# lucidrains/audiolm-pytorch

Hardware: NVIDIA H100
Metric: CoarseTransformer tokens/sec fwd+bwd seq2048 (higher is better)
Workload: dtype bf16

## Files before the change

### audiolm_pytorch_b200/_lib.py

```python
from __future__ import annotations

import ctypes as C
import os
from pathlib import Path

import torch

_PKG = Path(__file__).resolve().parent
LIB_PATH = _PKG / "libalm_b200.so"

P = C.c_void_p
I = C.c_int
L = C.c_int64
F = C.c_float
U32 = C.c_uint32
U64 = C.c_uint64
DROP = [F, U64, U32]

SIGNATURES: dict[str, list] = {
    "alm_gemm_bf16": [P, I, L, L, P, I, L, L, P, I, L, L, I, I, I, I, F, P, I, I, P],
    "alm_mqa_attn_fwd": [P, L, P, L, L, P, L, L, P, P, L, P, L, P, L, L, I, I, I, I, I, F, *DROP, P],
    "alm_mqa_attn_bwd": [P, L, P, L, L, P, L, L, P, L, P, P, P, I, P, L, P, P, L, P, L, P, P, L, L, I, I, I, I, I, F, *DROP,
                         P],
    "alm_pack_key_mask": [P, P, I, I, P],
# ... 51 lines not shown
    "alm_sq_decode": [P, I, I, I, I, I, I, P, P, P, P, I, I, P, L, P],
    "alm_hubert_conv0": [P, P, P, P, I, I, I, I, I, P],
    "alm_hubert_chan_stats": [P, P, I, I, I, P],
    "alm_hubert_norm_act": [P, P, I, P, L, P, P, I, P, P, L, I, P],
    "alm_hubert_add_ln": [P, P, I, I, P, I, P, P, I, P, P, L, I, P],
    "alm_hubert_pos_pack": [P, P, I, I, I, I, I, I, P],
    "alm_hubert_qkv_heads": [P, P, P, P, I, I, I, I, P],
    "alm_hubert_merge_heads": [P, P, I, I, I, I, P],
}


class AlmError(RuntimeError):
    pass


_lib = None


def load() -> C.CDLL:
    global _lib
    if _lib is not None:
        return _lib
    if not LIB_PATH.exists():
        raise AlmError(
            f"{LIB_PATH} not found. Build it with `python -m audiolm_pytorch_b200.build` "
            "(there is no CPU / PyTorch fallback for the hot path)."
        )
    lib = C.CDLL(str(LIB_PATH), mode=os.RTLD_LOCAL | os.RTLD_NOW)
    lib.alm_version.restype = I
    lib.alm_status_string.restype = C.c_char_p
    lib.alm_status_string.argtypes = [I]
    lib.alm_launch_count.restype = C.c_ulonglong
    lib.alm_reset_launch_count.restype = None
    lib.alm_decode_stack_scratch_bytes.restype = L
    lib.alm_decode_stack_scratch_bytes.argtypes = [I, I, I, I]
    lib.alm_gemm_head_ce_tiles.restype = I
    lib.alm_gemm_head_ce_tiles.argtypes = [I]
    lib.alm_codec_gate_loop_workspace.restype = C.c_longlong
    lib.alm_codec_gate_loop_workspace.argtypes = [I, I, I, I]
    lib.alm_decode_stack_grid.restype = I
    lib.alm_decode_stack_grid.argtypes = []
    lib.alm_decode_stack_plan.restype = I
    lib.alm_decode_stack_plan.argtypes = [I, I, I, I, I, P]
    lib.alm_decode_stack_plan_dh.restype = I
    lib.alm_decode_stack_plan_dh.argtypes = [I, I, I, I, I, I, P]
    lib.alm_decode_stack_trace_offset.restype = L
    lib.alm_decode_stack_trace_offset.argtypes = [I, I, I, I]
    for name, argtypes in SIGNATURES.items():
        fn = getattr(lib, name)
        fn.argtypes = argtypes
        fn.restype = I
    _lib = lib
    return lib


def ptr(t) -> int | None:
    if t is None:
        return None
    return t.data_ptr()


def stream_handle() -> int:
    return torch.cuda.current_stream().cuda_stream


def call(name: str, *args) -> None:
    lib = load()
    conv = []
    for a in args:
        if isinstance(a, torch.Tensor):
            if not a.is_cuda:
                raise AlmError(f"{name}: got a {a.device} tensor; the hot path has no CPU implementation")
            conv.append(a.data_ptr())
        else:
            conv.append(a)
    rc = getattr(lib, name)(*conv, stream_handle())
    if rc != 0:
        raise AlmError(f"{name} failed: {lib.alm_status_string(rc).decode()} ({rc})")


def launch_count() -> int:
    return int(load().alm_launch_count())


def reset_launch_count() -> None:
    load().alm_reset_launch_count()
```

### audiolm_pytorch_b200/csrc/ffn_loss_misc.cu

```cuda
#include <stdlib.h>

#include "alm_common.cuh"

namespace alm {

constexpr int FF_THREADS = 256;
constexpr int FF_MAX_CHUNKS = 4;

__device__ __forceinline__ void unpack8b(const uint4& u, float (&f)[8]) {
  f[0] = bf16_lo(u.x); f[1] = bf16_hi(u.x); f[2] = bf16_lo(u.y); f[3] = bf16_hi(u.y);
  f[4] = bf16_lo(u.z); f[5] = bf16_hi(u.z); f[6] = bf16_lo(u.w); f[7] = bf16_hi(u.w);
}
__device__ __forceinline__ uint32_t pk2b(float a, float b) {
  __nv_bfloat162 v = __floats2bfloat162_rn(a, b);
  return *reinterpret_cast<uint32_t*>(&v);
}
__device__ __forceinline__ uint4 pack8b(const float (&f)[8]) {
  return make_uint4(pk2b(f[0], f[1]), pk2b(f[2], f[3]), pk2b(f[4], f[5]), pk2b(f[6], f[7]));
}

template <int N>
__device__ __forceinline__ void block_sum256(float (&v)[N], float* buf ) {
  const int lane = threadIdx.x & 31, warp = threadIdx.x >> 5;
#pragma unroll
  for (int i = 0; i < N; ++i) v[i] = warp_sum(v[i]);
  __syncthreads();
  if (lane == 0) {
#pragma unroll
    for (int i = 0; i < N; ++i) buf[i * 8 + warp] = v[i];
  }
  __syncthreads();
#pragma unroll
  for (int i = 0; i < N; ++i) {
    float s = 0.f;
#pragma unroll
// ... 17 lines not shown
#pragma unroll
  for (int i = 0; i < N; ++i) {
    float s = 0.f;
#pragma unroll
    for (int w = 0; w < NW; ++w) s += buf[i * NW + w];
    v[i] = s;
  }
}

__device__ __forceinline__ uint32_t row_keep_bits8(const DropoutArgs& d, uint32_t m, uint32_t c0) {
  const uint32_t hi = (c0 >> 3) & 1u;
  const uint32_t jb = c0 & ~15u;
  uint32_t own[4], other[4];
#pragma unroll
  for (int t = 0; t < 4; ++t) {
    own[t] = dropout_word(dropout_draw(d, m, jb + 4 * hi + t), m);
    other[t] = __shfl_xor_sync(0xffffffffu, own[t], 1);
  }
  uint32_t bits = 0;
#pragma unroll
  for (int e = 0; e < 8; ++e) {
    const uint32_t w = ((uint32_t)e >> 2) == hi ? own[e & 3] : other[e & 3];
    if (dropout_pick(d, make_uint4(w, w, w, w), m, c0 + e)) bits |= 1u << e;
  }
  return bits;
}

__device__ __forceinline__ float gelu_erf(float x) { return 0.5f * x * (1.f + erff(x * 0.7071067811865476f)); }

__device__ __forceinline__ float gelu_erf_grad(float x) {
  const float cdf = 0.5f * (1.f + erff(x * 0.7071067811865476f));
  const float pdf = 0.3989422804014327f * __expf(-0.5f * x * x);
  return cdf + x * pdf;
}

template <int NCH, int NT, bool DROPOUT>
__global__ void __launch_bounds__(NT)
geglu_ln_fwd_kernel(const __nv_bfloat16* __restrict__ h, long long ldh, int gate_off,
                    const float* __restrict__ gamma, __nv_bfloat16* __restrict__ gn, long long ldg,
                    float* __restrict__ stats, int M, int inner, int inner_pad, const DropoutArgs drop) {
  __shared__ float buf[2 * (NT / 32)];
  uint4 pa[NCH], pgt[NCH];
  auto load_row = [&](int row, uint4* xa, uint4* xg) {
#pragma unroll
    for (int k = 0; k < NCH; ++k) {
      const int c0 = (threadIdx.x + k * NT) * 8;
      if (c0 < inner_pad) {
        xa[k] = *reinterpret_cast<const uint4*>(h + (size_t)row * ldh + c0);
        xg[k] = *reinterpret_cast<const uint4*>(h + (size_t)row * ldh + gate_off + c0);
      }
    }
  };
  if ((int)blockIdx.x < M) load_row(blockIdx.x, pa, pgt);
  for (int m = blockIdx.x; m < M; m += gridDim.x) {
    uint4 na[NCH], ngt[NCH];
    if (m + (int)gridDim.x < M) load_row(m + gridDim.x, na, ngt);
    if (m + 2 * (int)gridDim.x < M && (threadIdx.x & 7) == 0) {
#pragma unroll
      for (int k = 0; k < NCH; ++k) {
        const int c0 = (threadIdx.x + k * NT) * 8;
        if (c0 < inner_pad) {
          asm volatile("prefetch.global.L2 [%0];" ::"l"(h + (size_t)(m + 2 * gridDim.x) * ldh + c0));
          asm volatile("prefetch.global.L2 [%0];" ::"l"(h + (size_t)(m + 2 * gridDim.x) * ldh + gate_off + c0));
        }
      }
    }
    float g[NCH][8];
    float s12[2] = {0.f, 0.f};
#pragma unroll
    for (int k = 0; k < NCH; ++k) {
      const int c0 = (threadIdx.x + k * NT) * 8;
#pragma unroll
      for (int e = 0; e < 8; ++e) g[k][e] = 0.f;
      if (c0 < inner_pad) {
        float a[8], gt[8];
        unpack8b(pa[k], a);
        unpack8b(pgt[k], gt);
        const int nv = min(8, inner - c0);
#pragma unroll
        for (int e = 0; e < 8; ++e) {
          float cdf, xpdf;
          gelu_parts(gt[e], cdf, xpdf);
          const float v = e < nv ? gt[e] * cdf * a[e] : 0.f;
          g[k][e] = v;
          s12[0] += v;
          s12[1] = fmaf(v, v, s12[1]);
        }
      }
    }
    block_sum_nt<2, NT>(s12, buf);
    const float mean = s12[0] / inner;
    const float rstd = rsqrtf(fmaxf(s12[1] / inner - mean * mean, 0.f) + 1e-5f);
#pragma unroll
    for (int k = 0; k < NCH; ++k) {
      const int c0 = (threadIdx.x + k * NT) * 8;
      [[maybe_unused]] uint32_t keep = 0;
      if constexpr (DROPOUT) keep = row_keep_bits8(drop, m, c0);
      if (c0 < inner_pad) {
        const int nv = min(8, inner - c0);
        float gm[8] = {0.f, 0.f, 0.f, 0.f, 0.f, 0.f, 0.f, 0.f};
        if (nv == 8) {
          const float4 g0 = __ldg(reinterpret_cast<const float4*>(gamma + c0));
          const float4 g1 = __ldg(reinterpret_cast<const float4*>(gamma + c0 + 4));
          gm[0] = g0.x; gm[1] = g0.y; gm[2] = g0.z; gm[3] = g0.w; gm[4] = g1.x; gm[5] = g1.y; gm[6] = g1.z; gm[7] = g1.w;
        } else {
#pragma unroll
          for (int e = 0; e < 8; ++e)
            if (e < nv) gm[e] = __ldg(gamma + c0 + e);
        }
        float o[8];
#pragma unroll
        for (int e = 0; e < 8; ++e) o[e] = e < nv ? (g[k][e] - mean) * rstd * gm[e] : 0.f;
        if constexpr (DROPOUT) {
#pragma unroll
          for (int e = 0; e < 8; ++e) o[e] = ((keep >> e) & 1u) ? o[e] * drop.scale : 0.f;
        }
        *reinterpret_cast<uint4*>(gn + (size_t)m * ldg + c0) = pack8b(o);
      }
    }
    if (threadIdx.x == 0) {
      stats[(size_t)m * 2] = mean;
      stats[(size_t)m * 2 + 1] = rstd;
    }
#pragma unroll
    for (int k = 0; k < NCH; ++k) { pa[k] = na[k]; pgt[k] = ngt[k]; }
  }
}

template <int NCH, int NT, bool DROPOUT>
__global__ void __launch_bounds__(NT, NT == 512 ? 2 : 1)
geglu_ln_bwd_kernel(const __nv_bfloat16* __restrict__ h, long long ldh, int gate_off,
                    const float* __restrict__ gamma, const float* __restrict__ stats,
                    const __nv_bfloat16* __restrict__ dgn, long long ldg, __nv_bfloat16* __restrict__ dh,
                    float* __restrict__ g_gamma, int M, int inner, int inner_pad, const DropoutArgs drop) {
  __shared__ float buf[2 * (NT / 32)];
  float gacc[NCH][8];
#pragma unroll
  for (int k = 0; k < NCH; ++k)
#pragma unroll
    for (int e = 0; e < 8; ++e) gacc[k][e] = 0.f;
  for (int m = blockIdx.x; m < M; m += gridDim.x) {
    if (m + (int)gridDim.x < M && (threadIdx.x & 7) == 0) {
#pragma unroll
      for (int k = 0; k < NCH; ++k) {
        const int c0 = (threadIdx.x + k * NT) * 8;
        if (c0 < inner_pad) {
          asm volatile("prefetch.global.L2 [%0];" ::"l"(h + (size_t)(m + gridDim.x) * ldh + c0));
          asm volatile("prefetch.global.L2 [%0];" ::"l"(h + (size_t)(m + gridDim.x) * ldh + gate_off + c0));
          asm volatile("prefetch.global.L2 [%0];" ::"l"(dgn + (size_t)(m + gridDim.x) * ldg + c0));
        }
      }
    }
    const float mean = stats[(size_t)m * 2], rstd = stats[(size_t)m * 2 + 1];
    float a[NCH][8], gp[NCH][8], gl[NCH][8], ge[NCH][8];
    float r2[2] = {0.f, 0.f};
#pragma unroll
    for (int k = 0; k < NCH; ++k) {
      const int c0 = (threadIdx.x + k * NT) * 8;
#pragma unroll
      for (int e = 0; e < 8; ++e) { a[k][e] = gp[k][e] = gl[k][e] = ge[k][e] = 0.f; }
      [[maybe_unused]] uint32_t keep = 0;
      if constexpr (DROPOUT) keep = row_keep_bits8(drop, m, c0);
      if (c0 < inner_pad) {
        float dv[8], gt[8];
        unpack8b(*reinterpret_cast<const uint4*>(h + (size_t)m * ldh + c0), a[k]);
        unpack8b(*reinterpret_cast<const uint4*>(h + (size_t)m * ldh + gate_off + c0), gt);
        unpack8b(*reinterpret_cast<const uint4*>(dgn + (size_t)m * ldg + c0), dv);
        if constexpr (DROPOUT) {
#pragma unroll
          for (int e = 0; e < 8; ++e) dv[e] = ((keep >> e) & 1u) ? dv[e] * drop.scale : 0.f;
        }
        const int nv = min(8, inner - c0);
        float gm[8] = {0.f, 0.f, 0.f, 0.f, 0.f, 0.f, 0.f, 0.f};
        if (nv == 8) {
          const float4 g0 = __ldg(reinterpret_cast<const float4*>(gamma + c0));
          const float4 g1 = __ldg(reinterpret_cast<const float4*>(gamma + c0 + 4));
          gm[0] = g0.x; gm[1] = g0.y; gm[2] = g0.z; gm[3] = g0.w; gm[4] = g1.x; gm[5] = g1.y; gm[6] = g1.z; gm[7] = g1.w;
        } else {
#pragma unroll
          for (int e = 0; e < 8; ++e)
            if (e < nv) gm[e] = __ldg(gamma + c0 + e);
        }
#pragma unroll
        for (int e = 0; e < 8; ++e) {
          float cdf, xpdf;
          gelu_parts(gt[e], cdf, xpdf);
          const bool ok = e < nv;
          ge[k][e] = ok ? gt[e] * cdf : 0.f;
          gp[k][e] = ok ? cdf + xpdf : 0.f;
          if (!ok) { a[k][e] = 0.f; dv[e] = 0.f; }
          const float xh = (ge[k][e] * a[k][e] - mean) * rstd;
          gl[k][e] = dv[e] * gm[e];
          gacc[k][e] = fmaf(dv[e], xh, gacc[k][e]);
          r2[0] += gl[k][e];
          r2[1] = fmaf(gl[k][e], xh, r2[1]);
        }
      }
    }
    block_sum_nt<2, NT>(r2, buf);
    const float m1 = r2[0] / inner, m2 = r2[1] / inner;
#pragma unroll
    for (int k = 0; k < NCH; ++k) {
      const int c0 = (threadIdx.x + k * NT) * 8;
      if (c0 < inner_pad) {
        const int nv = min(8, inner - c0);
        float da[8], dg8[8];
#pragma unroll
        for (int e = 0; e < 8; ++e) {
          const float xh = (ge[k][e] * a[k][e] - mean) * rstd;
          const float dg = e < nv ? rstd * (gl[k][e] - m1 - xh * m2) : 0.f;
          da[e] = dg * ge[k][e];
          dg8[e] = dg * a[k][e] * gp[k][e];
        }
        *reinterpret_cast<uint4*>(dh + (size_t)m * ldh + c0) = pack8b(da);
        *reinterpret_cast<uint4*>(dh + (size_t)m * ldh + gate_off + c0) = pack8b(dg8);
      }
    }
  }
#pragma unroll
  for (int k = 0; k < NCH; ++k) {
    const int c0 = (threadIdx.x + k * NT) * 8;
#pragma unroll
    for (int e = 0; e < 8; ++e)
      if (c0 + e < inner) atomicAdd(g_gamma + c0 + e, gacc[k][e]);
  }
}



__global__ void __launch_bounds__(FF_THREADS)
ce_fwd_bwd_kernel(const float* __restrict__ logits, long long ldl, const long long* __restrict__ labels,
                  long long ignore_index, float* __restrict__ loss_rows, __nv_bfloat16* __restrict__ dlogits,
                  long long ldd, const float* __restrict__ scale_num, const float* __restrict__ scale_den, int V,
                  int Vpad) {
  __shared__ float buf[2 * 8];
  const int r = blockIdx.x;
  const float* row = logits + (size_t)r * ldl;
  const long long label = labels[r];
  const bool ignored = (label == ignore_index);
  const bool bad_label = !ignored && (label < 0 || label >= V);
  float mx[1] = {-INFINITY};
  for (int c = threadIdx.x; c < V; c += FF_THREADS) mx[0] = fmaxf(mx[0], row[c]);
  {
    float v = warp_max(mx[0]);
    __syncthreads();
    if ((threadIdx.x & 31) == 0) buf[threadIdx.x >> 5] = v;
    __syncthreads();
    float m = buf[0];
#pragma unroll
    for (int w = 1; w < FF_THREADS / 32; ++w) m = fmaxf(m, buf[w]);
    mx[0] = m;
  }
  float sm[1] = {0.f};
  for (int c = threadIdx.x; c < V; c += FF_THREADS) sm[0] += __expf(row[c] - mx[0]);
  block_sum256<1>(sm, buf);
  const float lse = mx[0] + logf(sm[0]);
  const float nan = __int_as_float(0x7fc00000);
  if (threadIdx.x == 0) loss_rows[r] = ignored ? 0.f : bad_label ? nan : (lse - row[label]);
  if (dlogits != nullptr) {
    const float sc = ignored ? 0.f : bad_label ? nan : (*scale_num) / (*scale_den);
// ... 246 lines not shown
#pragma unroll
    for (int half = 0; half < 2; ++half) {
      const uint32_t c = j0 + 8 * half;
      if ((int)c >= C) continue;
      uint4* ptr = reinterpret_cast<uint4*>(x + (size_t)row * ld + c);
      float f[8];
      unpack8b(*ptr, f);
#pragma unroll
      for (int e = 0; e < 8; ++e) f[e] = dropout_pick(d, dr[e], row, c + e) ? f[e] * d.scale : 0.f;
      *ptr = pack8b(f);
    }
  }
}

}

using namespace alm;

extern "C" int alm_dropout_bf16(void* x, int64_t ld, int64_t M, int C, float p, uint64_t seed, uint32_t site,
                                alm_stream_t stream_) {
  cudaStream_t stream = reinterpret_cast<cudaStream_t>(stream_);
  ALM_REQUIRE(x && M >= 0 && C >= 0 && p >= 0.f && p < 1.f, ALM_ERR_ARG);
  ALM_REQUIRE(C % 8 == 0 && ld % 8 == 0 && ld >= C && (reinterpret_cast<uintptr_t>(x) & 15u) == 0, ALM_ERR_ALIGN);
  ALM_REQUIRE(M < (1ll << 32), ALM_ERR_UNSUPPORTED);
  if (M == 0 || C == 0 || p == 0.f) return ALM_OK;
  const long long threads = (M + 15) / 16 * 4 * ((C + 15) / 16);
  dropout_bf16_kernel<<<(unsigned)ceil_div(threads, 256LL), 256, 0, stream>>>(
      reinterpret_cast<__nv_bfloat16*>(x), ld, M, C, make_dropout_args(p, seed, site));
  ALM_CHECK_LAUNCH();
  ALM_LAUNCHED(1);
  return ALM_OK;
}

template <bool DROPOUT>
static void launch_geglu_ln_fwd(int nch, int grid, cudaStream_t stream, const __nv_bfloat16* hp, int64_t ldh,
                                int gate_off, const float* gamma, __nv_bfloat16* gp, int64_t ldg, float* stats, int M,
                                int inner, int inner_pad, const DropoutArgs& d) {
  if (nch <= 1) geglu_ln_fwd_kernel<1, 256, DROPOUT><<<grid, FF_THREADS, 0, stream>>>(hp, ldh, gate_off, gamma, gp, ldg, stats, M, inner, inner_pad, d);
  else if (nch == 2) geglu_ln_fwd_kernel<2, 256, DROPOUT><<<grid, FF_THREADS, 0, stream>>>(hp, ldh, gate_off, gamma, gp, ldg, stats, M, inner, inner_pad, d);
  else geglu_ln_fwd_kernel<4, 256, DROPOUT><<<grid, FF_THREADS, 0, stream>>>(hp, ldh, gate_off, gamma, gp, ldg, stats, M, inner, inner_pad, d);
}

extern "C" int alm_geglu_ln_fwd(const void* h, int64_t ldh, int gate_off, const float* gamma, void* gn, int64_t ldg,
                                float* stats, int M, int inner, int inner_pad, float dropout_p, uint64_t seed,
                                uint32_t site, alm_stream_t stream_) {
  cudaStream_t stream = reinterpret_cast<cudaStream_t>(stream_);
  ALM_REQUIRE(M > 0 && inner > 0 && inner_pad >= inner && inner_pad % 8 == 0, ALM_ERR_ARG);
  ALM_REQUIRE(dropout_p >= 0.f && dropout_p < 1.f, ALM_ERR_ARG);
  ALM_REQUIRE(ldh % 8 == 0 && ldg % 8 == 0 && gate_off % 8 == 0, ALM_ERR_ALIGN);
  const int nch = ceil_div(inner_pad / 8, FF_THREADS);
  ALM_REQUIRE(nch <= FF_MAX_CHUNKS, ALM_ERR_UNSUPPORTED);
  const int grid = min(M, num_sms() * 8);
  auto* hp = (const __nv_bfloat16*)h;
  auto* gp = (__nv_bfloat16*)gn;
  const DropoutArgs d = make_dropout_args(dropout_p, seed, site);
  if (dropout_p > 0.f) launch_geglu_ln_fwd<true>(nch, grid, stream, hp, ldh, gate_off, gamma, gp, ldg, stats, M, inner, inner_pad, d);
  else launch_geglu_ln_fwd<false>(nch, grid, stream, hp, ldh, gate_off, gamma, gp, ldg, stats, M, inner, inner_pad, d);
  ALM_CHECK_LAUNCH();
  ALM_LAUNCHED(1);
  return ALM_OK;
}

template <bool DROPOUT>
static void launch_geglu_ln_bwd(int nch, int threads, int grid, cudaStream_t stream, const __nv_bfloat16* hp,
                                int64_t ldh, int gate_off, const float* gamma, const float* stats,
                                const __nv_bfloat16* dg, int64_t ldg, __nv_bfloat16* dhp, float* g_gamma, int M,
                                int inner, int inner_pad, const DropoutArgs& d) {
  if (threads == 512) geglu_ln_bwd_kernel<1, 512, DROPOUT><<<grid, 512, 0, stream>>>(hp, ldh, gate_off, gamma, stats, dg, ldg, dhp, g_gamma, M, inner, inner_pad, d);
  else if (nch <= 1) geglu_ln_bwd_kernel<1, 256, DROPOUT><<<grid, FF_THREADS, 0, stream>>>(hp, ldh, gate_off, gamma, stats, dg, ldg, dhp, g_gamma, M, inner, inner_pad, d);
  else if (nch == 2) geglu_ln_bwd_kernel<2, 256, DROPOUT><<<grid, FF_THREADS, 0, stream>>>(hp, ldh, gate_off, gamma, stats, dg, ldg, dhp, g_gamma, M, inner, inner_pad, d);
  else geglu_ln_bwd_kernel<4, 256, DROPOUT><<<grid, FF_THREADS, 0, stream>>>(hp, ldh, gate_off, gamma, stats, dg, ldg, dhp, g_gamma, M, inner, inner_pad, d);
}

extern "C" int alm_geglu_ln_bwd(const void* h, int64_t ldh, int gate_off, const float* gamma, const float* stats,
                                const void* dgn, int64_t ldg, void* dh, float* g_gamma, int M, int inner,
                                int inner_pad, float dropout_p, uint64_t seed, uint32_t site, alm_stream_t stream_) {
  cudaStream_t stream = reinterpret_cast<cudaStream_t>(stream_);
  ALM_REQUIRE(M > 0 && inner > 0 && inner_pad >= inner && inner_pad % 8 == 0, ALM_ERR_ARG);
  ALM_REQUIRE(dropout_p >= 0.f && dropout_p < 1.f, ALM_ERR_ARG);
  ALM_REQUIRE(ldh % 8 == 0 && ldg % 8 == 0 && gate_off % 8 == 0, ALM_ERR_ALIGN);
  const int nch = ceil_div(inner_pad / 8, FF_THREADS);
  ALM_REQUIRE(nch <= FF_MAX_CHUNKS, ALM_ERR_UNSUPPORTED);
  auto* hp = (const __nv_bfloat16*)h;
  auto* dg = (const __nv_bfloat16*)dgn;
  auto* dhp = (__nv_bfloat16*)dh;
  static const int bwd_threads = getenv("ALM_GEGLU_BWD_THREADS") ? atoi(getenv("ALM_GEGLU_BWD_THREADS")) : 512;
  const int threads = bwd_threads == 512 && inner_pad > 2048 && inner_pad <= 4096 ? 512 : 256;
  const int grid = min(M, num_sms() * (threads == 512 ? 2 : 4));
  const DropoutArgs d = make_dropout_args(dropout_p, seed, site);
  if (dropout_p > 0.f) launch_geglu_ln_bwd<true>(nch, threads, grid, stream, hp, ldh, gate_off, gamma, stats, dg, ldg, dhp, g_gamma, M, inner, inner_pad, d);
  else launch_geglu_ln_bwd<false>(nch, threads, grid, stream, hp, ldh, gate_off, gamma, stats, dg, ldg, dhp, g_gamma, M, inner, inner_pad, d);
  ALM_CHECK_LAUNCH();
  ALM_LAUNCHED(1);
  return ALM_OK;
}

extern "C" int alm_ce_fwd_bwd(const float* logits, int64_t ldl, const int64_t* labels, int64_t ignore_index,
                              float* loss_rows, void* dlogits, int64_t ldd, const float* scale_num,
                              const float* scale_den, int rows, int V, int Vpad, alm_stream_t stream_) {
  cudaStream_t stream = reinterpret_cast<cudaStream_t>(stream_);
  ALM_REQUIRE(rows > 0 && V > 0 && Vpad >= V, ALM_ERR_ARG);
  ALM_REQUIRE(dlogits == nullptr || (scale_num && scale_den), ALM_ERR_ARG);
  ce_fwd_bwd_kernel<<<rows, FF_THREADS, 0, stream>>>(logits, ldl, (const long long*)labels, ignore_index,
                                                    loss_rows, (__nv_bfloat16*)dlogits, ldd, scale_num, scale_den, V,
                                                    Vpad);
  ALM_CHECK_LAUNCH();
  ALM_LAUNCHED(1);
  return ALM_OK;
}

extern "C" int alm_attn_delta_dh(const void* o, int64_t ldo, const void* d_o, int64_t lddo, float* delta,
                                 int64_t delta_stride, float* dq_acc, int b, int h, int n, int dim_head,
                                 alm_stream_t stream_) {
  cudaStream_t stream = reinterpret_cast<cudaStream_t>(stream_);
  ALM_REQUIRE(dim_head == 32 || dim_head == 64 || dim_head == 128, ALM_ERR_UNSUPPORTED);
  ALM_REQUIRE(b > 0 && h > 0 && n > 0, ALM_ERR_ARG);
  const long long warps = (long long)b * h * n;
  const int threads = 256;
  const long long blocks = ceil_div(warps * 32, (long long)threads);
  attn_delta_kernel<<<(unsigned)blocks, threads, 0, stream>>>((const __nv_bfloat16*)o, ldo,
                                                              (const __nv_bfloat16*)d_o, lddo, delta, delta_stride, dq_acc, b, h, n,
                                                              dim_head);
  ALM_CHECK_LAUNCH();
  ALM_LAUNCHED(1);
  return ALM_OK;
}

extern "C" int alm_attn_delta(const void* o, int64_t ldo, const void* d_o, int64_t lddo, float* delta,
// ... 128 lines not shown
```

### include/alm_b200.h

```cpp
#ifndef ALM_B200_H_
#define ALM_B200_H_

#include <stddef.h>
#include <stdint.h>

#ifdef __cplusplus
extern "C" {
#endif

typedef struct CUstream_st* alm_stream_t;

typedef enum alm_status {
  ALM_OK = 0,
  ALM_ERR_ARG = -1,
  ALM_ERR_ALIGN = -2,
  ALM_ERR_CUDA = -3,
  ALM_ERR_UNSUPPORTED = -4
} alm_status;

int alm_version(void);
const char* alm_status_string(int code);
unsigned long long alm_launch_count(void);
void alm_reset_launch_count(void);

// ... 78 lines not shown
                          float scale, int grid_ctas , alm_stream_t stream);

int alm_hc_pre_fwd(const void* R_in, const void* Y, const float* beta_prev, const float* x_expand,
                   const float* gamma_hc, const float* dyn_alpha, const float* dyn_beta, const float* static_alpha,
                   const float* static_beta, const float* alpha_scale, const float* beta_scale,
                   const float* ln_gamma, void* R_out, void* bin, void* xn, float* beta_out, float* aux, int M,
                   int d, int streams, alm_stream_t stream);
int alm_hc_pre_bwd(const void* R_in, const void* Y, const float* beta_prev, const float* x_expand,
                   const float* gamma_hc, const float* dyn_alpha, const float* dyn_beta, const float* static_alpha,
                   const float* static_beta, const float* alpha_scale, const float* beta_scale,
                   const float* ln_gamma, const float* aux, const void* dR_out, const void* dxn,
                   const void* dbin_extra, const float* dbeta, void* dR_in, void* dY, float* dbeta_prev,
                   float* dx_expand, float dx_scale, float* g_gamma_hc, float* g_dyn_alpha, float* g_dyn_beta,
                   float* g_static_alpha, float* g_static_beta, float* g_alpha_scale, float* g_beta_scale,
                   float* g_ln_gamma, int M, int d, int streams, alm_stream_t stream);
int alm_hc_post_fwd(const void* R_in, const void* Y, const float* beta_prev, const float* ln_gamma, void* out,
                    float* stats, int M, int d, int streams, alm_stream_t stream);
int alm_hc_post_bwd(const void* R_in, const void* Y, const float* beta_prev, const float* ln_gamma,
                    const float* stats, const void* dout, void* dR_in, void* dY, float* dbeta_prev,
                    float* g_ln_gamma, int M, int d, int streams, alm_stream_t stream);

int alm_resid_ln_fwd(const float* r, const void* y, const float* gamma, float* r_new, void* xn, void* rb, float* stats,
                     int M, int d, alm_stream_t stream);
int alm_resid_ln_bwd(const float* r_new, const float* gamma, const float* stats, const float* dr_out, const void* dxn,
                     const void* dextra, float* dr, void* dr_bf16, float* g_gamma, float out_scale, int M, int d,
                     alm_stream_t stream);

int alm_geglu_ln_fwd(const void* h, int64_t ldh, int gate_off, const float* gamma, void* gn, int64_t ldg,
                     float* stats, int M, int inner, int inner_pad, float dropout_p, uint64_t seed, uint32_t site,
                     alm_stream_t stream);
int alm_geglu_ln_bwd(const void* h, int64_t ldh, int gate_off, const float* gamma, const float* stats,
                     const void* dgn, int64_t ldg, void* dh, float* g_gamma, int M, int inner, int inner_pad,
                     float dropout_p, uint64_t seed, uint32_t site, alm_stream_t stream);

int alm_dropout_bf16(void* x, int64_t ld, int64_t M, int C, float p, uint64_t seed, uint32_t site,
                     alm_stream_t stream);

int alm_ce_fwd_bwd(const float* logits, int64_t ldl, const int64_t* labels, int64_t ignore_index, float* loss_rows,
                   void* dlogits, int64_t ldd, const float* scale_num, const float* scale_den, int rows, int V,
                   int Vpad, alm_stream_t stream);

int alm_topk_gumbel_sample(const float* logits, int64_t ldl, const float* uniform, int64_t ldu, int64_t* ids, int rows,
                           int V, int k, float temperature, alm_stream_t stream);

int alm_axpby_bf16(const void* x, int64_t ldx, float alpha, const void* y, int64_t ldy, float beta, void* out,
                   int64_t ldout, int64_t rows, int cols, alm_stream_t stream);
int alm_cast_pad_bf16(const float* src, int64_t lds, void* dst, int64_t ldd, int64_t rows, int cols, int cols_pad,
                      alm_stream_t stream);
int alm_cast_pad_multi(const int64_t* desc_dev, int n, alm_stream_t stream);
int alm_scale_by_scalar_bf16(void* x, const float* s, int64_t n, alm_stream_t stream);

int alm_causal_conv1d_fwd(const float* x, const float* w, const float* bias, const float* residual, float* y, int B,
                          int Cin, int Cout, int T, int K, int stride, int dilation, int pad_mode, int act_elu,
                          int w_packed, alm_stream_t stream);
int alm_residual_unit_fwd(const float* x, const float* w7_packed, const float* b7, const float* w1_packed,
                          const float* b1, float* y, int B, int C, int T, int dilation, int pad_mode,
                          alm_stream_t stream);
int alm_codec_se_fp32(const float* y, const float* x, const float* w1_folded, const float* b1, const float* w2,
                      const float* b2, float* out, int B, int C, int Ci, int T, alm_stream_t stream);
int alm_codec_first_conv(const float* x, const float* w, const float* bias, void* y, int B, int T, int Cout, int K,
                         int pad_mode, alm_stream_t stream);
int alm_codec_ru_tc(const void* x, void* y, const void* w_units, const float* b7, const float* b1, int B, int C, int T,
                    int dilation, int pad_mode, int out_phases, alm_stream_t stream);
int alm_codec_conv_tc(const void* x, void* y, const void* w_units, const float* bias, int B, int Cin, int Cout, int Tin,
                      int K, int stride, int pad_mode, int out_phases, int out_fp32, int upsample, alm_stream_t stream);
int alm_codec_ru_se_tc(const void* x, void* y, const void* w_units, const float* b7, const float* b1, const float* se_b1,
// ... 50 lines not shown
```

Before: 743,500.

## Add TMA bulk-copy ring-buffered persistent kernels for GEGLU+LayerNorm fwd/bwd

Adds persistent GEGLU+LayerNorm forward and backward kernels. Each prefetches whole input rows into a multi-stage shared-memory ring with cp.async.bulk and mbarriers, so the next rows' loads overlap compute on the current row. The old register-load kernels are refactored into shared device helpers and kept as a fallback, used for wide rows, small M, misaligned bases, or when an env var disables the ring. The ring adds shared-memory pressure and limits CTAs per SM, and a launch counter is exposed for inspection.

```diff
diff --git a/audiolm_pytorch_b200/_lib.py b/audiolm_pytorch_b200/_lib.py
--- a/audiolm_pytorch_b200/_lib.py
+++ b/audiolm_pytorch_b200/_lib.py
@@ -107,6 +107,7 @@
     lib.alm_status_string.argtypes = [I]
     lib.alm_launch_count.restype = C.c_ulonglong
     lib.alm_reset_launch_count.restype = None
+    lib.alm_geglu_ring_launches.restype = C.c_ulonglong
     lib.alm_decode_stack_scratch_bytes.restype = L
     lib.alm_decode_stack_scratch_bytes.argtypes = [I, I, I, I]
     lib.alm_gemm_head_ce_tiles.restype = I
@@ -160,3 +161,7 @@
 
 def reset_launch_count() -> None:
     load().alm_reset_launch_count()
+
+
+def geglu_ring_launches() -> int:
+    return int(load().alm_geglu_ring_launches())
diff --git a/audiolm_pytorch_b200/csrc/ffn_loss_misc.cu b/audiolm_pytorch_b200/csrc/ffn_loss_misc.cu
--- a/audiolm_pytorch_b200/csrc/ffn_loss_misc.cu
+++ b/audiolm_pytorch_b200/csrc/ffn_loss_misc.cu
@@ -1,6 +1,10 @@
 #include <stdlib.h>
+#include <string.h>
+
+#include <initializer_list>
 
 #include "alm_common.cuh"
+#include "ptx_sm90.cuh"
 
 namespace alm {
 
@@ -84,6 +88,103 @@
   const float cdf = 0.5f * (1.f + erff(x * 0.7071067811865476f));
   const float pdf = 0.3989422804014327f * __expf(-0.5f * x * x);
   return cdf + x * pdf;
+}
+
+
+__device__ __forceinline__ void load_gamma8(const float* __restrict__ gamma, int c0, int nv, float (&gm)[8]) {
+#pragma unroll
+  for (int e = 0; e < 8; ++e) gm[e] = 0.f;
+  if (nv == 8) {
+    const float4 g0 = __ldg(reinterpret_cast<const float4*>(gamma + c0));
+    const float4 g1 = __ldg(reinterpret_cast<const float4*>(gamma + c0 + 4));
+    gm[0] = g0.x; gm[1] = g0.y; gm[2] = g0.z; gm[3] = g0.w; gm[4] = g1.x; gm[5] = g1.y; gm[6] = g1.z; gm[7] = g1.w;
+  } else {
+#pragma unroll
+    for (int e = 0; e < 8; ++e)
+      if (e < nv) gm[e] = __ldg(gamma + c0 + e);
+  }
+}
+
+__device__ __forceinline__ void geglu_fwd_chunk(const uint4& ua, const uint4& ugt, int nv, float (&g)[8],
+                                                float (&s12)[2]) {
+  float a[8], gt[8];
+  unpack8b(ua, a);
+  unpack8b(ugt, gt);
+#pragma unroll
+  for (int e = 0; e < 8; ++e) {
+    float cdf, xpdf;
+    gelu_parts(gt[e], cdf, xpdf);
+    const float v = e < nv ? gt[e] * cdf * a[e] : 0.f;
+    g[e] = v;
+    s12[0] += v;
+    s12[1] = fmaf(v, v, s12[1]);
+  }
+}
+
+__device__ __forceinline__ void geglu_ln_stats(const float (&s12)[2], int inner, float& mean, float& rstd) {
+  mean = s12[0] / inner;
+  rstd = rsqrtf(fmaxf(fmaf(-mean, mean, s12[1] / inner), 0.f) + 1e-5f);
+}
+
+template <bool DROPOUT>
+__device__ __forceinline__ uint4 geglu_fwd_out(const float (&g)[8], const float* __restrict__ gamma, int c0, int nv,
+                                               float mean, float rstd, uint32_t keep, const DropoutArgs& drop) {
+  float gm[8];
+  load_gamma8(gamma, c0, nv, gm);
+  float o[8];
+#pragma unroll
+  for (int e = 0; e < 8; ++e) o[e] = e < nv ? (g[e] - mean) * rstd * gm[e] : 0.f;
+  if constexpr (DROPOUT) {
+#pragma unroll
+    for (int e = 0; e < 8; ++e) o[e] = ((keep >> e) & 1u) ? o[e] * drop.scale : 0.f;
+  }
+  return pack8b(o);
+}
+
+template <bool DROPOUT>
+__device__ __forceinline__ void geglu_bwd_chunk(const uint4& ua, const uint4& ugt, const uint4& udg, uint32_t keep,
+                                                const float* __restrict__ gamma, int c0, int nv, float mean,
+                                                float rstd, const DropoutArgs& drop, float (&a)[8], float (&ge)[8],
+                                                float (&gp)[8], float (&gl)[8], float (&gacc)[8], float (&r2)[2]) {
+  float dv[8], gt[8];
+  unpack8b(ua, a);
+  unpack8b(ugt, gt);
+  unpack8b(udg, dv);
+  if constexpr (DROPOUT) {
+#pragma unroll
+    for (int e = 0; e < 8; ++e) dv[e] = ((keep >> e) & 1u) ? dv[e] * drop.scale : 0.f;
+  }
+  float gm[8];
+  load_gamma8(gamma, c0, nv, gm);
+#pragma unroll
+  for (int e = 0; e < 8; ++e) {
+    float cdf, xpdf;
+    gelu_parts(gt[e], cdf, xpdf);
+    const bool ok = e < nv;
+    ge[e] = ok ? gt[e] * cdf : 0.f;
+    gp[e] = ok ? cdf + xpdf : 0.f;
+    if (!ok) { a[e] = 0.f; dv[e] = 0.f; }
+    const float xh = (ge[e] * a[e] - mean) * rstd;
+    gl[e] = dv[e] * gm[e];
+    gacc[e] = fmaf(dv[e], xh, gacc[e]);
+    r2[0] += gl[e];
+    r2[1] = fmaf(gl[e], xh, r2[1]);
+  }
+}
+
+__device__ __forceinline__ void geglu_bwd_out(const float (&a)[8], const float (&ge)[8], const float (&gp)[8],
+                                              const float (&gl)[8], int nv, float mean, float rstd, float m1, float m2,
+                                              uint4& da_out, uint4& dgt_out) {
+  float da[8], dg8[8];
+#pragma unroll
+  for (int e = 0; e < 8; ++e) {
+    const float xh = (ge[e] * a[e] - mean) * rstd;
+    const float dg = e < nv ? rstd * (gl[e] - m1 - xh * m2) : 0.f;
+    da[e] = dg * ge[e];
+    dg8[e] = dg * a[e] * gp[e];
+  }
+  da_out = pack8b(da);
+  dgt_out = pack8b(dg8);
 }
 
 template <int NCH, int NT, bool DROPOUT>
@@ -124,51 +225,19 @@
       const int c0 = (threadIdx.x + k * NT) * 8;
 #pragma unroll
       for (int e = 0; e < 8; ++e) g[k][e] = 0.f;
-      if (c0 < inner_pad) {
-        float a[8], gt[8];
-        unpack8b(pa[k], a);
-        unpack8b(pgt[k], gt);
-        const int nv = min(8, inner - c0);
-#pragma unroll
-        for (int e = 0; e < 8; ++e) {
-          float cdf, xpdf;
-          gelu_parts(gt[e], cdf, xpdf);
-          const float v = e < nv ? gt[e] * cdf * a[e] : 0.f;
-          g[k][e] = v;
-          s12[0] += v;
-          s12[1] = fmaf(v, v, s12[1]);
-        }
-      }
+      if (c0 < inner_pad) geglu_fwd_chunk(pa[k], pgt[k], min(8, inner - c0), g[k], s12);
     }
     block_sum_nt<2, NT>(s12, buf);
-    const float mean = s12[0] / inner;
-    const float rstd = rsqrtf(fmaxf(s12[1] / inner - mean * mean, 0.f) + 1e-5f);
+    float mean, rstd;
+    geglu_ln_stats(s12, inner, mean, rstd);
 #pragma unroll
     for (int k = 0; k < NCH; ++k) {
       const int c0 = (threadIdx.x + k * NT) * 8;
       [[maybe_unused]] uint32_t keep = 0;
       if constexpr (DROPOUT) keep = row_keep_bits8(drop, m, c0);
-      if (c0 < inner_pad) {
-        const int nv = min(8, inner - c0);
-        float gm[8] = {0.f, 0.f, 0.f, 0.f, 0.f, 0.f, 0.f, 0.f};
-        if (nv == 8) {
-          const float4 g0 = __ldg(reinterpret_cast<const float4*>(gamma + c0));
-          const float4 g1 = __ldg(reinterpret_cast<const float4*>(gamma + c0 + 4));
-          gm[0] = g0.x; gm[1] = g0.y; gm[2] = g0.z; gm[3] = g0.w; gm[4] = g1.x; gm[5] = g1.y; gm[6] = g1.z; gm[7] = g1.w;
-        } else {
-#pragma unroll
-          for (int e = 0; e < 8; ++e)
-            if (e < nv) gm[e] = __ldg(gamma + c0 + e);
-        }
-        float o[8];
-#pragma unroll
-        for (int e = 0; e < 8; ++e) o[e] = e < nv ? (g[k][e] - mean) * rstd * gm[e] : 0.f;
-        if constexpr (DROPOUT) {
-#pragma unroll
-          for (int e = 0; e < 8; ++e) o[e] = ((keep >> e) & 1u) ? o[e] * drop.scale : 0.f;
-        }
-        *reinterpret_cast<uint4*>(gn + (size_t)m * ldg + c0) = pack8b(o);
-      }
+      if (c0 < inner_pad)
+        *reinterpret_cast<uint4*>(gn + (size_t)m * ldg + c0) =
+            geglu_fwd_out<DROPOUT>(g[k], gamma, c0, min(8, inner - c0), mean, rstd, keep, drop);
     }
     if (threadIdx.x == 0) {
       stats[(size_t)m * 2] = mean;
@@ -213,60 +282,21 @@
       for (int e = 0; e < 8; ++e) { a[k][e] = gp[k][e] = gl[k][e] = ge[k][e] = 0.f; }
       [[maybe_unused]] uint32_t keep = 0;
       if constexpr (DROPOUT) keep = row_keep_bits8(drop, m, c0);
-      if (c0 < inner_pad) {
-        float dv[8], gt[8];
-        unpack8b(*reinterpret_cast<const uint4*>(h + (size_t)m * ldh + c0), a[k]);
-        unpack8b(*reinterpret_cast<const uint4*>(h + (size_t)m * ldh + gate_off + c0), gt);
-        unpack8b(*reinterpret_cast<const uint4*>(dgn + (size_t)m * ldg + c0), dv);
-        if constexpr (DROPOUT) {
-#pragma unroll
-          for (int e = 0; e < 8; ++e) dv[e] = ((keep >> e) & 1u) ? dv[e] * drop.scale : 0.f;
-        }
-        const int nv = min(8, inner - c0);
-        float gm[8] = {0.f, 0.f, 0.f, 0.f, 0.f, 0.f, 0.f, 0.f};
-        if (nv == 8) {
-          const float4 g0 = __ldg(reinterpret_cast<const float4*>(gamma + c0));
-          const float4 g1 = __ldg(reinterpret_cast<const float4*>(gamma + c0 + 4));
-          gm[0] = g0.x; gm[1] = g0.y; gm[2] = g0.z; gm[3] = g0.w; gm[4] = g1.x; gm[5] = g1.y; gm[6] = g1.z; gm[7] = g1.w;
-        } else {
-#pragma unroll
-          for (int e = 0; e < 8; ++e)
-            if (e < nv) gm[e] = __ldg(gamma + c0 + e);
-        }
-#pragma unroll
-        for (int e = 0; e < 8; ++e) {
-          float cdf, xpdf;
-          gelu_parts(gt[e], cdf, xpdf);
-          const bool ok = e < nv;
-          ge[k][e] = ok ? gt[e] * cdf : 0.f;
-          gp[k][e] = ok ? cdf + xpdf : 0.f;
-          if (!ok) { a[k][e] = 0.f; dv[e] = 0.f; }
-          const float xh = (ge[k][e] * a[k][e] - mean) * rstd;
-          gl[k][e] = dv[e] * gm[e];
-          gacc[k][e] = fmaf(dv[e], xh, gacc[k][e]);
-          r2[0] += gl[k][e];
-          r2[1] = fmaf(gl[k][e], xh, r2[1]);
-        }
-      }
+      if (c0 < inner_pad)
+        geglu_bwd_chunk<DROPOUT>(*reinterpret_cast<const uint4*>(h + (size_t)m * ldh + c0),
+                                 *reinterpret_cast<const uint4*>(h + (size_t)m * ldh + gate_off + c0),
+                                 *reinterpret_cast<const uint4*>(dgn + (size_t)m * ldg + c0), keep, gamma, c0,
+                                 min(8, inner - c0), mean, rstd, drop, a[k], ge[k], gp[k], gl[k], gacc[k], r2);
     }
     block_sum_nt<2, NT>(r2, buf);
     const float m1 = r2[0] / inner, m2 = r2[1] / inner;
 #pragma unroll
     for (int k = 0; k < NCH; ++k) {
       const int c0 = (threadIdx.x + k * NT) * 8;
-      if (c0 < inner_pad) {
-        const int nv = min(8, inner - c0);
-        float da[8], dg8[8];
-#pragma unroll
-        for (int e = 0; e < 8; ++e) {
-          const float xh = (ge[k][e] * a[k][e] - mean) * rstd;
-          const float dg = e < nv ? rstd * (gl[k][e] - m1 - xh * m2) : 0.f;
-          da[e] = dg * ge[k][e];
-          dg8[e] = dg * a[k][e] * gp[k][e];
-        }
-        *reinterpret_cast<uint4*>(dh + (size_t)m * ldh + c0) = pack8b(da);
-        *reinterpret_cast<uint4*>(dh + (size_t)m * ldh + gate_off + c0) = pack8b(dg8);
-      }
+      if (c0 < inner_pad)
+        geglu_bwd_out(a[k], ge[k], gp[k], gl[k], min(8, inner - c0), mean, rstd, m1, m2,
+                      *reinterpret_cast<uint4*>(dh + (size_t)m * ldh + c0),
+                      *reinterpret_cast<uint4*>(dh + (size_t)m * ldh + gate_off + c0));
     }
   }
 #pragma unroll
@@ -278,6 +308,167 @@
   }
 }
 
+constexpr int RING_FWD_NT = 256, RING_FWD_NCH = 2;
+constexpr int RING_FWD_CTAS = 4, RING_FWD_STAGES = 3;
+constexpr int RING_BWD_NT = 512;
+constexpr int RING_BWD_CTAS = 2, RING_BWD_STAGES = 3;
+constexpr int RING_MAX_INNER_PAD = RING_FWD_NT * RING_FWD_NCH * 8;
+static_assert(RING_MAX_INNER_PAD == RING_BWD_NT * 8, "the two ring kernels cover the same rows");
+constexpr int RING_MIN_ROWS_PER_SM = 4;
+
+__host__ __device__ inline int ring_stage_bytes(int rows, int inner_pad) { return (rows * 2 * inner_pad + 127) / 128 * 128; }
+
+template <int NST>
+__device__ __forceinline__ void ring_init(uint64_t (&full)[NST]) {
+  if (threadIdx.x == 0) {
+    for (int i = 0; i < NST; ++i) mbar_init(&full[i], 1);
+    fence_mbar_init();
+  }
+  __syncthreads();
+}
+
+template <int NST>
+__device__ __forceinline__ void ring_advance(int& ls, uint32_t& phase) {
+  if (++ls == NST) {
+    ls = 0;
+    phase ^= 1;
+  }
+}
+
+template <bool DROPOUT>
+__global__ void __launch_bounds__(RING_FWD_NT, RING_FWD_CTAS)
+geglu_ln_fwd_ring(const __nv_bfloat16* __restrict__ h, long long ldh, int gate_off, const float* __restrict__ gamma,
+                  __nv_bfloat16* __restrict__ gn, long long ldg, float* __restrict__ stats, int M, int inner,
+                  int inner_pad, const DropoutArgs drop) {
+  constexpr int NT = RING_FWD_NT, NCH = RING_FWD_NCH, NST = RING_FWD_STAGES;
+  extern __shared__ __align__(128) unsigned char ring[];
+  __shared__ uint64_t full[NST];
+  __shared__ float buf[2 * (NT / 32)];
+  const uint32_t row_b = 2u * inner_pad;
+  const int stage_b = ring_stage_bytes(2, inner_pad);
+  auto fill = [&](int k) {
+    const int m = blockIdx.x + k * gridDim.x;
+    if (m >= M) return;
+    unsigned char* st = ring + (size_t)(k % NST) * stage_b;
+    uint64_t* bar = &full[k % NST];
+    mbar_arrive_expect_tx(bar, 2 * row_b);
+    bulk_copy_g2s(st, h + (size_t)m * ldh, row_b, bar);
+    bulk_copy_g2s(st + row_b, h + (size_t)m * ldh + gate_off, row_b, bar);
+  };
+  ring_init(full);
+  if (threadIdx.x == 0)
+    for (int k = 0; k < NST; ++k) fill(k);
+  int ls = 0;
+  uint32_t phase = 0;
+  for (int k = 0, m = blockIdx.x; m < M; ++k, m += gridDim.x) {
+    const unsigned char* st = ring + (size_t)ls * stage_b;
+    mbar_wait(&full[ls], phase);
+    float g[NCH][8];
+    float s12[2] = {0.f, 0.f};
+#pragma unroll
+    for (int c = 0; c < NCH; ++c) {
+      const int c0 = (threadIdx.x + c * NT) * 8;
+#pragma unroll
+      for (int e = 0; e < 8; ++e) g[c][e] = 0.f;
+      if (c0 < inner_pad)
+        geglu_fwd_chunk(*reinterpret_cast<const uint4*>(st + 2 * c0),
+                        *reinterpret_cast<const uint4*>(st + row_b + 2 * c0), min(8, inner - c0), g[c], s12);
+    }
+    block_sum_nt<2, NT>(s12, buf);
+    if (threadIdx.x == 0) {
+      fence_proxy_async_smem();
+      fill(k + NST);
+    }
+    float mean, rstd;
+    geglu_ln_stats(s12, inner, mean, rstd);
+#pragma unroll
+    for (int c = 0; c < NCH; ++c) {
+      const int c0 = (threadIdx.x + c * NT) * 8;
+      [[maybe_unused]] uint32_t keep = 0;
+      if constexpr (DROPOUT) keep = row_keep_bits8(drop, m, c0);
+      if (c0 < inner_pad)
+        *reinterpret_cast<uint4*>(gn + (size_t)m * ldg + c0) =
+            geglu_fwd_out<DROPOUT>(g[c], gamma, c0, min(8, inner - c0), mean, rstd, keep, drop);
+    }
+    if (threadIdx.x == 0) {
+      stats[(size_t)m * 2] = mean;
+      stats[(size_t)m * 2 + 1] = rstd;
+    }
+    ring_advance<NST>(ls, phase);
+  }
+}
+
+template <bool DROPOUT>
+__global__ void __launch_bounds__(RING_BWD_NT, RING_BWD_CTAS)
+geglu_ln_bwd_ring(const __nv_bfloat16* __restrict__ h, long long ldh, int gate_off, const float* __restrict__ gamma,
+                  const float* __restrict__ stats, const __nv_bfloat16* __restrict__ dgn, long long ldg,
+                  __nv_bfloat16* __restrict__ dh, float* __restrict__ g_gamma, int M, int inner, int inner_pad,
+                  const DropoutArgs drop) {
+  constexpr int NT = RING_BWD_NT, NST = RING_BWD_STAGES;
+  extern __shared__ __align__(128) unsigned char ring[];
+  __shared__ uint64_t full[NST];
+  __shared__ float buf[2 * (NT / 32)];
+  const uint32_t row_b = 2u * inner_pad;
+  const int stage_b = ring_stage_bytes(3, inner_pad);
+  auto fill = [&](int k) {
+    const int m = blockIdx.x + k * gridDim.x;
+    if (m >= M) return;
+    unsigned char* st = ring + (size_t)(k % NST) * stage_b;
+    uint64_t* bar = &full[k % NST];
+    mbar_arrive_expect_tx(bar, 3 * row_b);
+    bulk_copy_g2s(st, h + (size_t)m * ldh, row_b, bar);
+    bulk_copy_g2s(st + row_b, h + (size_t)m * ldh + gate_off, row_b, bar);
+    bulk_copy_g2s(st + 2 * row_b, dgn + (size_t)m * ldg, row_b, bar);
+  };
+  ring_init(full);
+  if (threadIdx.x == 0)
+    for (int k = 0; k < NST; ++k) fill(k);
+  const int c0 = threadIdx.x * 8;
+  const int nv = min(8, inner - c0);
+  float gacc[8];
+#pragma unroll
+  for (int e = 0; e < 8; ++e) gacc[e] = 0.f;
+  float nmean = 0.f, nrstd = 0.f;
+  if ((int)blockIdx.x < M) {
+    nmean = stats[(size_t)blockIdx.x * 2];
+    nrstd = stats[(size_t)blockIdx.x * 2 + 1];
+  }
+  int ls = 0;
+  uint32_t phase = 0;
+  for (int k = 0, m = blockIdx.x; m < M; ++k, m += gridDim.x) {
+    const float mean = nmean, rstd = nrstd;
+    if (m + (int)gridDim.x < M) {
+      nmean = stats[(size_t)(m + gridDim.x) * 2];
+      nrstd = stats[(size_t)(m + gridDim.x) * 2 + 1];
+    }
+    const unsigned char* st = ring + (size_t)ls * stage_b;
+    [[maybe_unused]] uint32_t keep = 0;
+    if constexpr (DROPOUT) keep = row_keep_bits8(drop, m, c0);
+    float a[8], gp[8], gl[8], ge[8];
+    float r2[2] = {0.f, 0.f};
+#pragma unroll
+    for (int e = 0; e < 8; ++e) { a[e] = gp[e] = gl[e] = ge[e] = 0.f; }
+    mbar_wait(&full[ls], phase);
+    if (c0 < inner_pad)
+      geglu_bwd_chunk<DROPOUT>(*reinterpret_cast<const uint4*>(st + 2 * c0),
+                               *reinterpret_cast<const uint4*>(st + row_b + 2 * c0),
+                               *reinterpret_cast<const uint4*>(st + 2 * row_b + 2 * c0), keep, gamma, c0, nv, mean,
+                               rstd, drop, a, ge, gp, gl, gacc, r2);
+    block_sum_nt<2, NT>(r2, buf);
+    if (threadIdx.x == 0) {
+      fence_proxy_async_smem();
+      fill(k + NST);
+    }
+    const float m1 = r2[0] / inner, m2 = r2[1] / inner;
+    if (c0 < inner_pad)
+      geglu_bwd_out(a, ge, gp, gl, nv, mean, rstd, m1, m2, *reinterpret_cast<uint4*>(dh + (size_t)m * ldh + c0),
+                    *reinterpret_cast<uint4*>(dh + (size_t)m * ldh + gate_off + c0));
+    ring_advance<NST>(ls, phase);
+  }
+#pragma unroll
+  for (int e = 0; e < 8; ++e)
+    if (c0 + e < inner) atomicAdd(g_gamma + c0 + e, gacc[e]);
+}
 
 
 __global__ void __launch_bounds__(FF_THREADS)
@@ -590,6 +781,50 @@
   return ALM_OK;
 }
 
+static unsigned long long g_geglu_ring_launches = 0;
+
+static bool geglu_ring_ok(int M, int inner_pad, std::initializer_list<const void*> bases) {
+  static const bool enabled = [] {
+    const char* v = getenv("ALM_GEGLU_RING");
+    return !(v && strcmp(v, "0") == 0);
+  }();
+  if (!enabled || inner_pad > RING_MAX_INNER_PAD || M < RING_MIN_ROWS_PER_SM * num_sms()) return false;
+  for (const void* p : bases)
+    if (reinterpret_cast<uintptr_t>(p) & 15u) return false;
+  return true;
+}
+
+template <auto K>
+static cudaError_t ring_opt_in(int bytes) {
+  static const cudaError_t err = cudaFuncSetAttribute(K, cudaFuncAttributeMaxDynamicSharedMemorySize, bytes);
+  return err;
+}
+
+template <bool DROPOUT>
+static cudaError_t launch_geglu_fwd_ring(cudaStream_t stream, const __nv_bfloat16* hp, int64_t ldh, int gate_off,
+                                         const float* gamma, __nv_bfloat16* gp, int64_t ldg, float* stats, int M,
+                                         int inner, int inner_pad, const DropoutArgs& d) {
+  constexpr auto K = geglu_ln_fwd_ring<DROPOUT>;
+  const cudaError_t e = ring_opt_in<K>(RING_FWD_STAGES * ring_stage_bytes(2, RING_MAX_INNER_PAD));
+  if (e != cudaSuccess) return e;
+  K<<<min(M, num_sms() * RING_FWD_CTAS), RING_FWD_NT, RING_FWD_STAGES * ring_stage_bytes(2, inner_pad), stream>>>(
+      hp, ldh, gate_off, gamma, gp, ldg, stats, M, inner, inner_pad, d);
+  return cudaSuccess;
+}
+
+template <bool DROPOUT>
+static cudaError_t launch_geglu_bwd_ring(cudaStream_t stream, const __nv_bfloat16* hp, int64_t ldh, int gate_off,
+                                         const float* gamma, const float* stats, const __nv_bfloat16* dg, int64_t ldg,
+                                         __nv_bfloat16* dhp, float* g_gamma, int M, int inner, int inner_pad,
+                                         const DropoutArgs& d) {
+  constexpr auto K = geglu_ln_bwd_ring<DROPOUT>;
+  const cudaError_t e = ring_opt_in<K>(RING_BWD_STAGES * ring_stage_bytes(3, RING_MAX_INNER_PAD));
+  if (e != cudaSuccess) return e;
+  K<<<min(M, num_sms() * RING_BWD_CTAS), RING_BWD_NT, RING_BWD_STAGES * ring_stage_bytes(3, inner_pad), stream>>>(
+      hp, ldh, gate_off, gamma, stats, dg, ldg, dhp, g_gamma, M, inner, inner_pad, d);
+  return cudaSuccess;
+}
+
 template <bool DROPOUT>
 static void launch_geglu_ln_fwd(int nch, int grid, cudaStream_t stream, const __nv_bfloat16* hp, int64_t ldh,
                                 int gate_off, const float* gamma, __nv_bfloat16* gp, int64_t ldg, float* stats, int M,
@@ -608,12 +843,18 @@
   ALM_REQUIRE(ldh % 8 == 0 && ldg % 8 == 0 && gate_off % 8 == 0, ALM_ERR_ALIGN);
   const int nch = ceil_div(inner_pad / 8, FF_THREADS);
   ALM_REQUIRE(nch <= FF_MAX_CHUNKS, ALM_ERR_UNSUPPORTED);
-  const int grid = min(M, num_sms() * 8);
   auto* hp = (const __nv_bfloat16*)h;
   auto* gp = (__nv_bfloat16*)gn;
   const DropoutArgs d = make_dropout_args(dropout_p, seed, site);
-  if (dropout_p > 0.f) launch_geglu_ln_fwd<true>(nch, grid, stream, hp, ldh, gate_off, gamma, gp, ldg, stats, M, inner, inner_pad, d);
-  else launch_geglu_ln_fwd<false>(nch, grid, stream, hp, ldh, gate_off, gamma, gp, ldg, stats, M, inner, inner_pad, d);
+  if (geglu_ring_ok(M, inner_pad, {h})) {
+    ALM_CUDA_OK(dropout_p > 0.f ? launch_geglu_fwd_ring<true>(stream, hp, ldh, gate_off, gamma, gp, ldg, stats, M, inner, inner_pad, d)
+                                : launch_geglu_fwd_ring<false>(stream, hp, ldh, gate_off, gamma, gp, ldg, stats, M, inner, inner_pad, d));
+    ++g_geglu_ring_launches;
+  } else {
+    const int grid = min(M, num_sms() * 8);
+    if (dropout_p > 0.f) launch_geglu_ln_fwd<true>(nch, grid, stream, hp, ldh, gate_off, gamma, gp, ldg, stats, M, inner, inner_pad, d);
+    else launch_geglu_ln_fwd<false>(nch, grid, stream, hp, ldh, gate_off, gamma, gp, ldg, stats, M, inner, inner_pad, d);
+  }
   ALM_CHECK_LAUNCH();
   ALM_LAUNCHED(1);
   return ALM_OK;
@@ -642,16 +883,26 @@
   auto* hp = (const __nv_bfloat16*)h;
   auto* dg = (const __nv_bfloat16*)dgn;
   auto* dhp = (__nv_bfloat16*)dh;
+  const DropoutArgs d = make_dropout_args(dropout_p, seed, site);
+  if (geglu_ring_ok(M, inner_pad, {h, dgn})) {
+    ALM_CUDA_OK(dropout_p > 0.f ? launch_geglu_bwd_ring<true>(stream, hp, ldh, gate_off, gamma, stats, dg, ldg, dhp, g_gamma, M, inner, inner_pad, d)
+                                : launch_geglu_bwd_ring<false>(stream, hp, ldh, gate_off, gamma, stats, dg, ldg, dhp, g_gamma, M, inner, inner_pad, d));
+    ++g_geglu_ring_launches;
+    ALM_CHECK_LAUNCH();
+    ALM_LAUNCHED(1);
+    return ALM_OK;
+  }
   static const int bwd_threads = getenv("ALM_GEGLU_BWD_THREADS") ? atoi(getenv("ALM_GEGLU_BWD_THREADS")) : 512;
   const int threads = bwd_threads == 512 && inner_pad > 2048 && inner_pad <= 4096 ? 512 : 256;
   const int grid = min(M, num_sms() * (threads == 512 ? 2 : 4));
-  const DropoutArgs d = make_dropout_args(dropout_p, seed, site);
   if (dropout_p > 0.f) launch_geglu_ln_bwd<true>(nch, threads, grid, stream, hp, ldh, gate_off, gamma, stats, dg, ldg, dhp, g_gamma, M, inner, inner_pad, d);
   else launch_geglu_ln_bwd<false>(nch, threads, grid, stream, hp, ldh, gate_off, gamma, stats, dg, ldg, dhp, g_gamma, M, inner, inner_pad, d);
   ALM_CHECK_LAUNCH();
   ALM_LAUNCHED(1);
   return ALM_OK;
 }
+
+extern "C" unsigned long long alm_geglu_ring_launches(void) { return g_geglu_ring_launches; }
 
 extern "C" int alm_ce_fwd_bwd(const float* logits, int64_t ldl, const int64_t* labels, int64_t ignore_index,
                               float* loss_rows, void* dlogits, int64_t ldd, const float* scale_num,
diff --git a/include/alm_b200.h b/include/alm_b200.h
--- a/include/alm_b200.h
+++ b/include/alm_b200.h
@@ -134,6 +134,7 @@
 int alm_geglu_ln_bwd(const void* h, int64_t ldh, int gate_off, const float* gamma, const float* stats,
                      const void* dgn, int64_t ldg, void* dh, float* g_gamma, int M, int inner, int inner_pad,
                      float dropout_p, uint64_t seed, uint32_t site, alm_stream_t stream);
+unsigned long long alm_geglu_ring_launches(void);
 
 int alm_dropout_bf16(void* x, int64_t ld, int64_t M, int C, float p, uint64_t seed, uint32_t site,
                      alm_stream_t stream);
```

After: 746,300 (median of 6 runs). Within noise of the previous version (+0.4%).
